# JinfengX/PointCloudPDF

Measured on AMD Instinct MI355X. Metric: points/sec fwd+bwd (PT-v1 Seg50 + PDF U-decoder, 100k-pt scenes), higher is better.
Workload: dtype f32

## Files before the change

### pointcloudpdf_amd/csrc/rowlin2_impl.h

```cpp
#pragma once
#include "pdfops_common.h"
#include <algorithm>
#include <cstdlib>

namespace rl2 {

typedef float f32x4 __attribute__((ext_vector_type(4)));

typedef _Float16 h16x4 __attribute__((ext_vector_type(4)));
typedef __bf16 b16x4 __attribute__((ext_vector_type(4)));
typedef short s16x4 __attribute__((ext_vector_type(4)));
template <int MP> struct Mma;
template <> struct Mma<0> {
    typedef f32x4 frag;
    static __device__ __forceinline__ frag cvt(f32x4 v) { return v; }
};
template <> struct Mma<1> {
    typedef h16x4 frag;
    static __device__ __forceinline__ frag cvt(f32x4 v) { return __builtin_convertvector(v, h16x4); }
    static __device__ __forceinline__ f32x4 mma(frag a, frag b, f32x4 acc) { return __builtin_amdgcn_mfma_f32_16x16x16f16(a, b, acc, 0, 0, 0); }
};
template <> struct Mma<2> {
    typedef s16x4 frag;
    static __device__ __forceinline__ frag cvt(f32x4 v) { return __builtin_bit_cast(s16x4, __builtin_convertvector(v, b16x4)); }
    static __device__ __forceinline__ f32x4 mma(frag a, frag b, f32x4 acc) { return __builtin_amdgcn_mfma_f32_16x16x16bf16_1k(a, b, acc, 0, 0, 0); }
};

long stats_rows_floats(long n, int o);

struct FwdArgs {
    long N;
    int O;
    const float *X[3]; long ldx;
    const float *W[3]; long wso, wsk;
    const float *bias[3];
    const float *scale, *shift; int relu;
    float *Y[3]; long ldy;
    int accumulate;
    float *partial;
    const float *bx; long ldb; const float *bcoef; int brelu;
    const float *roww; long rws;
    unsigned long long *ho_gran; unsigned *ho_sync;
};

constexpr int FWD_CAP = 1024;
static inline int fwd_row_blocks(long n) {
    const long tiles = (n + 15) / 16, b = (tiles + 3) / 4;
    return (int)(b < 1 ? 1 : (b > FWD_CAP ? FWD_CAP : b));
}

template <int K, int NOB, int NIN, bool PRE, int ST, int MP>
__global__ __launch_bounds__(256) void k_fwd(FwdArgs a) {
    typedef typename Mma<MP>::frag wfrag;
    constexpr bool STATS = ST != 0;
    constexpr int NJ = K / 16;
    constexpr bool COEF_REGS = K <= 64;
    const int lane = threadIdx.x & 63, wave = threadIdx.x >> 6;
    const int li = lane & 15, kq = lane >> 4;
    if (ST == 1 && a.ho_gran && blockIdx.x == 0 && blockIdx.y == 0) pdf_handoff_zero(a.ho_gran, a.O, a.ho_sync);
    const int gcol0 = blockIdx.y * NOB * 16;
    int outi[NOB], colb[NOB];
#pragma unroll
    for (int ob = 0; ob < NOB; ++ob) { outi[ob] = (gcol0 + ob * 16) / a.O; colb[ob] = gcol0 + ob * 16 - outi[ob] * a.O; }
    wfrag Wr[NIN][NOB][NJ];
#pragma unroll
    for (int in = 0; in < NIN; ++in) {
#pragma unroll
        for (int ob = 0; ob < NOB; ++ob) {
            const float *W = a.W[NIN > 1 ? in : outi[ob]];
            const long o = colb[ob] + li;
#pragma unroll
            for (int j = 0; j < NJ; ++j) {
                f32x4 w4;
                if (a.wsk == 1) {
                    w4 = *reinterpret_cast<const f32x4 *>(W + o * a.wso + 16 * j + 4 * kq);
                } else {
#pragma unroll
                    for (int c = 0; c < 4; ++c) w4[c] = W[o * a.wso + (long)(16 * j + 4 * kq + c) * a.wsk];
                }
                Wr[in][ob][j] = Mma<MP>::cvt(w4);
            }
        }
    }
    f32x4 bias4[NOB];
#pragma unroll
    for (int ob = 0; ob < NOB; ++ob) {
        const float *b = a.bias[NIN > 1 ? 0 : outi[ob]];
#pragma unroll
        for (int r = 0; r < 4; ++r) bias4[ob][r] = b ? b[colb[ob] + 4 * kq + r] : 0.f;
    }
    f32x4 sc4[COEF_REGS && PRE ? NJ : 1], sh4[COEF_REGS && PRE ? NJ : 1];
    if (PRE && COEF_REGS) {
#pragma unroll
        for (int j = 0; j < NJ; ++j) {
            sc4[j] = *reinterpret_cast<const f32x4 *>(a.scale + 16 * j + 4 * kq);
            sh4[j] = *reinterpret_cast<const f32x4 *>(a.shift + 16 * j + 4 * kq);
        }
    }
    f32x4 s4[STATS ? NOB : 1], ss4[STATS ? NOB : 1];
    if (STATS) {
#pragma unroll
        for (int ob = 0; ob < NOB; ++ob) { s4[ob] = f32x4{0.f, 0.f, 0.f, 0.f}; ss4[ob] = f32x4{0.f, 0.f, 0.f, 0.f}; }
    }
    __shared__ float bco[ST == 2 ? 3 : 1][NOB * 16];
    if (ST == 2) {
        if (threadIdx.x < 3 * NOB * 16) {
            const int v = threadIdx.x / (NOB * 16), t = threadIdx.x % (NOB * 16);
            bco[ST == 2 ? v : 0][t] = a.bcoef[(long)v * a.O + gcol0 + t];
        }
        __syncthreads();
    }
    __shared__ float pco[PRE && !COEF_REGS ? 2 : 1][PRE && !COEF_REGS ? K : 1];
    if (PRE && !COEF_REGS) {
        for (int t = threadIdx.x; t < K; t += 256) { pco[0][t] = a.scale[t]; pco[PRE && !COEF_REGS ? 1 : 0][t] = a.shift[t]; }
        __syncthreads();
    }
    const float relu_lo = a.relu ? 0.f : -INFINITY;
    constexpr int XB0 = NJ < 16 ? NJ : 16;
    constexpr int XB = (K == 256 && NIN == 3) ? 4 : ((ST != 0 && NOB > 1 && NIN * NOB * NJ * 4 >= 128) ? ((PRE && K == 128) ? 2 : XB0 / 2) : XB0);
    const long ntiles = (a.N + 15) / 16;
    for (long tile = (long)blockIdx.x * 4 + wave; tile < ntiles; tile += (long)gridDim.x * 4) {
        const long n = tile * 16 + li;
        const bool valid = n < a.N;
        f32x4 acc[NOB];
#pragma unroll
        for (int ob = 0; ob < NOB; ++ob) acc[ob] = f32x4{0.f, 0.f, 0.f, 0.f};
#pragma unroll
        for (int in = 0; in < NIN; ++in) {
            const float *xr = a.X[in] + (valid ? n : 0) * a.ldx + 4 * kq;
#pragma unroll
            for (int j0 = 0; j0 < NJ; j0 += XB) {
                f32x4 xb[XB];
#pragma unroll
                for (int t = 0; t < XB; ++t) xb[t] = *reinterpret_cast<const f32x4 *>(xr + 16 * (j0 + t));
                __builtin_amdgcn_sched_barrier(0);
#pragma unroll
                for (int t = 0; t < XB; ++t) {
                    const int j = j0 + t;
                    f32x4 x4 = xb[t];
                    if (PRE) {
                        const f32x4 sc = COEF_REGS ? sc4[COEF_REGS ? j : 0] : *reinterpret_cast<const f32x4 *>(&pco[0][16 * j + 4 * kq]);
                        const f32x4 sh = COEF_REGS ? sh4[COEF_REGS ? j : 0] : *reinterpret_cast<const f32x4 *>(&pco[PRE && !COEF_REGS ? 1 : 0][16 * j + 4 * kq]);
                        x4 = x4 * sc + sh;
#pragma unroll
                        for (int c = 0; c < 4; ++c) x4[c] = fmaxf(x4[c], relu_lo);
                    }
                    if constexpr (MP == 0) {
#pragma unroll
                        for (int c = 0; c < 4; ++c)
#pragma unroll
                            for (int ob = 0; ob < NOB; ++ob)
                                acc[ob] = __builtin_amdgcn_mfma_f32_16x16x4f32(Wr[in][ob][j][c], x4[c], acc[ob], 0, 0, 0);
                    } else {
                        const wfrag xh = Mma<MP>::cvt(x4);
#pragma unroll
                        for (int ob = 0; ob < NOB; ++ob) acc[ob] = Mma<MP>::mma(Wr[in][ob][j], xh, acc[ob]);
                    }
                }
            }
        }
#pragma unroll
        for (int ob = 0; ob < NOB; ++ob) {
            f32x4 v = acc[ob];
            if (a.roww) v *= a.roww[(valid ? n : 0) * a.rws];
            v += bias4[ob];
            float *dst = a.Y[outi[ob]] + (valid ? n : 0) * a.ldy + colb[ob] + 4 * kq;
            if (a.accumulate && valid) v += *reinterpret_cast<const f32x4 *>(dst);
            if (valid) *reinterpret_cast<f32x4 *>(dst) = v;
            if (ST == 1 && valid) { s4[ob] += v; ss4[ob] += v * v; }
            if (ST == 2) {
                const f32x4 x4 = *reinterpret_cast<const f32x4 *>(a.bx + (valid ? n : 0) * a.ldb + colb[ob] + 4 * kq);
                const f32x4 sc = *reinterpret_cast<const f32x4 *>(&bco[0][ob * 16 + 4 * kq]);
                const f32x4 sh = *reinterpret_cast<const f32x4 *>(&bco[ST == 2 ? 1 : 0][ob * 16 + 4 * kq]);
                const f32x4 mu = *reinterpret_cast<const f32x4 *>(&bco[ST == 2 ? 2 : 0][ob * 16 + 4 * kq]);
                const f32x4 pre = x4 * sc + sh;
                f32x4 gm;
#pragma unroll
                for (int c = 0; c < 4; ++c) gm[c] = (valid && (!a.brelu || pre[c] > 0.f)) ? v[c] : 0.f;
                s4[ob] += gm;
                ss4[ob] += gm * (x4 - mu);
            }
        }
    }
    if (STATS) {
        __shared__ float red[4][2][NOB * 16];
#pragma unroll
        for (int ob = 0; ob < NOB; ++ob)
#pragma unroll
            for (int r = 0; r < 4; ++r) {
                float s = s4[ob][r], ss = ss4[ob][r];
#pragma unroll
                for (int m = 1; m < 16; m <<= 1) { s += __shfl_xor(s, m, 64); ss += __shfl_xor(ss, m, 64); }
                if (li == 0) { red[wave][0][ob * 16 + 4 * kq + r] = s; red[wave][1][ob * 16 + 4 * kq + r] = ss; }
            }
        __syncthreads();
        const int t = threadIdx.x;
        if (t < NOB * 16) {
            float *row = a.partial + (size_t)blockIdx.x * 2 * a.O;
            row[gcol0 + t] = red[0][0][t] + red[1][0][t] + red[2][0][t] + red[3][0][t];
            const float ss = red[0][1][t] + red[1][1][t] + red[2][1][t] + red[3][1][t];
            row[a.O + gcol0 + t] = ST == 2 ? ss * a.bcoef[3 * (long)a.O + gcol0 + t] : ss;
        }
    }
}

constexpr int WG_MAXG = 5;
struct WArgs {
    long N;
    int K, O;
    const float *G[WG_MAXG]; long ldg;
    const float *X; long ldx;
    const float *scale, *shift; int relu;
    int per_z; const float *Xz[WG_MAXG]; const float *scalez[WG_MAXG], *shiftz[WG_MAXG]; int reluz[WG_MAXG];
    float *dW[WG_MAXG], *db[WG_MAXG];
    long rows_per_block;
    const float *roww; long rws;
    float *slab;
    float *bslab;
};

template <int VW> struct Vec;
template <> struct Vec<2> { typedef float type __attribute__((ext_vector_type(2))); };
template <> struct Vec<4> { typedef float type __attribute__((ext_vector_type(4))); };

template <int VW, bool PRE, bool RW, int MP>
__global__ __launch_bounds__(256) void k_wg(WArgs a) {
    typedef typename Vec<VW>::type vec;
    constexpr int B = 16 * VW;
    __shared__ float red[4][B * B];
    __shared__ float redb[4][B];
    const int lane = threadIdx.x & 63, wave = threadIdx.x >> 6;
    const int li = lane & 15, nq = lane >> 4;
    const int nkb = a.K / B;
    const int ob = (blockIdx.y / nkb) * B, kb = (blockIdx.y % nkb) * B;
    const float *G = a.G[blockIdx.z];
    const float *X = (PRE && a.per_z) ? a.Xz[blockIdx.z] : a.X;
    vec sc, sh;
    bool relu = a.relu != 0;
    if (PRE) {
        const float *scp = a.per_z ? a.scalez[blockIdx.z] : a.scale, *shp = a.per_z ? a.shiftz[blockIdx.z] : a.shift;
        if (a.per_z) relu = scp != nullptr && a.reluz[blockIdx.z] != 0;
        if (scp) {
            sc = *reinterpret_cast<const vec *>(scp + kb + VW * li);
            sh = *reinterpret_cast<const vec *>(shp + kb + VW * li);
        } else {
#pragma unroll
            for (int c = 0; c < VW; ++c) { sc[c] = 1.f; sh[c] = 0.f; }
        }
    }
    const float relu_lo = relu ? 0.f : -INFINITY;
    f32x4 acc[VW][VW];
    float gsum[VW];
#pragma unroll
    for (int c = 0; c < VW; ++c) {
        gsum[c] = 0.f;
#pragma unroll
        for (int c2 = 0; c2 < VW; ++c2) acc[c][c2] = f32x4{0.f, 0.f, 0.f, 0.f};
    }
    const long rb = (long)blockIdx.x * a.rows_per_block;
    const long re = rb + a.rows_per_block < a.N ? rb + a.rows_per_block : a.N;
    for (long r0 = rb + 16 * wave; r0 < re; r0 += 64) {
        vec gv[4], xv[4];
        float rw[RW ? 4 : 1];
        bool ok[4];
#pragma unroll
        for (int t = 0; t < 4; ++t) {
            const long n = r0 + 4 * t + nq;
            ok[t] = n < re;
            const long nn = ok[t] ? n : rb;
            gv[t] = *reinterpret_cast<const vec *>(G + nn * a.ldg + ob + VW * li);
            xv[t] = *reinterpret_cast<const vec *>(X + nn * a.ldx + kb + VW * li);
            if (RW) rw[RW ? t : 0] = a.roww[nn * a.rws];
        }
        __builtin_amdgcn_sched_barrier(0);
#pragma unroll
        for (int t = 0; t < 4; ++t) {
            if (RW) gv[t] *= rw[RW ? t : 0];
            if (PRE) {
                xv[t] = xv[t] * sc + sh;
#pragma unroll
                for (int c = 0; c < VW; ++c) xv[t][c] = fmaxf(xv[t][c], relu_lo);
            }
#pragma unroll
            for (int c = 0; c < VW; ++c) { gv[t][c] = ok[t] ? gv[t][c] : 0.f; xv[t][c] = ok[t] ? xv[t][c] : 0.f; }
        }
        if constexpr (MP == 0) {
#pragma unroll
            for (int t = 0; t < 4; ++t)
#pragma unroll
                for (int c = 0; c < VW; ++c) {
                    gsum[c] += gv[t][c];
#pragma unroll
                    for (int c2 = 0; c2 < VW; ++c2)
                        acc[c][c2] = __builtin_amdgcn_mfma_f32_16x16x4f32(gv[t][c], xv[t][c2], acc[c][c2], 0, 0, 0);
                }
        } else {
            typename Mma<MP>::frag ga[VW], xa[VW];
#pragma unroll
            for (int c = 0; c < VW; ++c) {
                gsum[c] += (gv[0][c] + gv[1][c]) + (gv[2][c] + gv[3][c]);
                ga[c] = Mma<MP>::cvt(f32x4{gv[0][c], gv[1][c], gv[2][c], gv[3][c]});
                xa[c] = Mma<MP>::cvt(f32x4{xv[0][c], xv[1][c], xv[2][c], xv[3][c]});
            }
#pragma unroll
            for (int c = 0; c < VW; ++c)
#pragma unroll
                for (int c2 = 0; c2 < VW; ++c2) acc[c][c2] = Mma<MP>::mma(ga[c], xa[c2], acc[c][c2]);
        }
    }
#pragma unroll
    for (int c = 0; c < VW; ++c)
#pragma unroll
        for (int c2 = 0; c2 < VW; ++c2)
#pragma unroll
            for (int r = 0; r < 4; ++r) red[wave][(VW * (4 * nq + r) + c) * B + VW * li + c2] = acc[c][c2][r];
    float *db = a.db[blockIdx.z];
    const bool want_db = db && kb == 0;
    if (want_db) {
#pragma unroll
        for (int c = 0; c < VW; ++c) {
            float g = gsum[c];
            g += __shfl_xor(g, 16, 64);
            g += __shfl_xor(g, 32, 64);
            if (nq == 0) redb[wave][VW * li + c] = g;
        }
    }
    __syncthreads();
    float *slab = a.slab + (((size_t)blockIdx.z * gridDim.y + blockIdx.y) * gridDim.x + blockIdx.x) * (B * B);
    for (int e = threadIdx.x; e < B * B; e += 256) slab[e] = (red[0][e] + red[1][e]) + (red[2][e] + red[3][e]);
    if (want_db && threadIdx.x < B)
        a.bslab[(((size_t)blockIdx.z * (a.O / B) + ob / B) * gridDim.x + blockIdx.x) * B + threadIdx.x] =
            (redb[0][threadIdx.x] + redb[1][threadIdx.x]) + (redb[2][threadIdx.x] + redb[3][threadIdx.x]);
}

struct RArgs {
    const float *slab, *bslab;
    float *dW[WG_MAXG], *db[WG_MAXG];
    int B, tiles_k, tiles, otiles, split, K, O;
};
void launch_slab_reduce(const RArgs &a, int ng, bool any_bias, hipStream_t s);
template <int L>
__global__ __launch_bounds__(64 * L) void k_slab_reduce(RArgs a) {
    __shared__ float red[L][64];
    const int e = threadIdx.x & 63, l = threadIdx.x >> 6, z = blockIdx.z;
    const int ei = blockIdx.x * 64 + e;
    const bool bias = (int)blockIdx.y >= a.tiles;
    const int t = bias ? (int)blockIdx.y - a.tiles : (int)blockIdx.y;
    const int len = bias ? a.B : a.B * a.B;
    if (bias && (int)blockIdx.x * 64 >= len) return;
    const float *src = bias ? a.bslab + ((size_t)z * a.otiles + t) * a.split * a.B : a.slab + ((size_t)z * a.tiles + t) * a.split * (size_t)(a.B * a.B);
    float s = 0.f;
    if (ei < len) {
        int k = l;
        for (; k + 3 * L < a.split; k += 4 * L) {
            const float v0 = src[(size_t)k * len + ei], v1 = src[(size_t)(k + L) * len + ei];
            const float v2 = src[(size_t)(k + 2 * L) * len + ei], v3 = src[(size_t)(k + 3 * L) * len + ei];
            s = (((s + v0) + v1) + v2) + v3;
        }
        for (; k < a.split; k += L) s += src[(size_t)k * len + ei];
    }
    red[l][e] = s;
    __syncthreads();
    if (l != 0 || ei >= len) return;
#pragma unroll
    for (int k = 1; k < L; ++k) s += red[k][e];
    if (bias) {
        const int o = t * a.B + ei;
        if (a.db[z] && o < a.O) a.db[z][o] = s;
    } else {
        const int o = (t / a.tiles_k) * a.B + ei / a.B, kk = (t % a.tiles_k) * a.B + ei % a.B;
        if (o < a.O && kk < a.K) a.dW[z][(size_t)o * a.K + kk] = s;
    }
}

#ifdef RL2_MAIN_TU
void launch_slab_reduce(const RArgs &a, int ng, bool any_bias, hipStream_t s) {
    const dim3 grid((unsigned)((a.B * a.B + 63) / 64), (unsigned)(a.tiles + (any_bias ? a.otiles : 0)), (unsigned)ng);
    if (a.split > 32) k_slab_reduce<16><<<grid, 64 * 16, 0, s>>>(a);
    else if (a.split > 4) k_slab_reduce<4><<<grid, 64 * 4, 0, s>>>(a);
    else k_slab_reduce<1><<<grid, 64, 0, s>>>(a);
}
#endif

struct WgPlan { int vw, b, nblk; long split, rows_per_block; };
static WgPlan wg_plan(long n, int k, int o, int ng) {
    WgPlan p;
    p.vw = (k % 64 == 0 && o % 64 == 0) ? 4 : ((k % 32 == 0 && o % 32 == 0) ? 2 : 0);
    p.b = 16 * p.vw;
    if (!p.vw) { p.nblk = 0; p.split = 0; p.rows_per_block = 0; return p; }
    p.nblk = (o / p.b) * (k / p.b) * ng;
    static const int target = [] { const char *v = getenv("PDFOPS_WG_BLOCKS"); const int x = v ? atoi(v) : 0; return x > 0 ? x : 512; }();
    long split = (target + p.nblk - 1) / p.nblk;
    const long max_split = (n + 255) / 256;
    if (split > max_split) split = max_split;
    if (split < 1) split = 1;
    p.rows_per_block = ((n + split - 1) / split + 63) / 64 * 64;
    p.split = (n + p.rows_per_block - 1) / p.rows_per_block;
    return p;
}
#ifdef RL2_MAIN_TU
long wgrad_ws_floats(long n, int k, int o, int ng) {
    const WgPlan p = wg_plan(n, k, o, ng);
    if (!p.vw) return 0;
    return (long)p.nblk * p.split * p.b * p.b + (long)ng * (o / p.b) * p.split * p.b;
}
#endif

static inline bool aligned16(const void *p) { return (reinterpret_cast<uintptr_t>(p) & 15) == 0; }

template <int K, int NOB, int NIN, int MP>
static int launch_fwd(const FwdArgs &a, int nslabs, hipStream_t s) {
    const bool pre = a.scale != nullptr, stats = a.partial != nullptr, bst = stats && a.bx != nullptr;
    static const int total = [] { const char *v = getenv("PDFOPS_RL_BLOCKS"); const int x = v ? atoi(v) : 0; return x > 0 ? x : 512; }();
    int gx = fwd_row_blocks(a.N);
    if (!stats || bst) gx = std::max(1, std::min(gx, std::max(8, total / std::max(nslabs, 1))));
    const dim3 grid((unsigned)gx, (unsigned)nslabs);
    if (bst) {
        k_fwd<K, NOB, NIN, false, 2, MP><<<grid, 256, 0, s>>>(a);
    } else if (NIN == 1 && stats) {
        if (pre) k_fwd<K, NOB, 1, true, 1, MP><<<grid, 256, 0, s>>>(a);
        else k_fwd<K, NOB, 1, false, 1, MP><<<grid, 256, 0, s>>>(a);
    } else {
        if (pre) k_fwd<K, NOB, NIN, true, 0, MP><<<grid, 256, 0, s>>>(a);
        else k_fwd<K, NOB, NIN, false, 0, MP><<<grid, 256, 0, s>>>(a);
    }
    return gx;
}

#ifdef RL2_MAIN_TU
long stats_rows_floats(long n, int o) { return (long)fwd_row_blocks(n) * 2 * o; }
#endif

template <int MP>
int try_forward_mp(long n, int k, int o, int nin, int nout, const float *const *x, long ldx, const float *const *w, int transpose_w,
                   const float *const *bias, const float *scale, const float *shift, int relu, float *const *y, long ldy,
                   int accumulate, float *partial, hipStream_t s, const float *roww, long rws, const float *bx, long ldb, const float *bcoef,
                   int brelu, int *partial_rows, long ldw, void *handoff) {
    if (nin < 1 || nout < 1 || (nin > 1 && nout > 1) || nin > 3 || nout > 3) return 0;
    if (nin == 2 && (scale || bx)) return 0;
    if (partial && !bx && (nin != 1 || nout != 1)) return 0;
    if (bx && (!partial || nout != 1 || scale || !bcoef || (ldb & 3) || !aligned16(bx) || !aligned16(bcoef))) return 0;
    if ((ldx & 3) || (ldy & 3) || (o & 15)) return 0;
    for (int i = 0; i < (nin > 1 ? nin : nout); ++i) if (!aligned16(w[i])) return 0;
    if (scale && (!aligned16(scale) || !aligned16(shift))) return 0;
    for (int i = 0; i < nin; ++i) if (!aligned16(x[i])) return 0;
    for (int i = 0; i < nout; ++i) if (!aligned16(y[i])) return 0;
    FwdArgs a;
    a.N = n; a.O = o; a.ldx = ldx; a.ldy = ldy; a.scale = scale; a.shift = shift; a.relu = relu; a.accumulate = accumulate;
    a.partial = partial; a.roww = roww; a.rws = rws;
    a.bx = bx; a.ldb = ldb; a.bcoef = bcoef; a.brelu = brelu;
    a.ho_gran = static_cast<unsigned long long *>(handoff);
    a.ho_sync = handoff ? reinterpret_cast<unsigned *>(a.ho_gran + 2 * (size_t)o) : nullptr;
    a.wso = transpose_w ? 1 : (ldw ? ldw : k); a.wsk = transpose_w ? o : 1;
    for (int i = 0; i < 3; ++i) {
        a.X[i] = i < nin ? x[i] : nullptr;
        a.W[i] = i < (nin > 1 ? nin : nout) ? w[i] : nullptr;
        a.bias[i] = (bias && i < nout) ? bias[i] : nullptr;
        a.Y[i] = i < nout ? y[i] : nullptr;
    }
    const int cols = o * nout;
#define PDF_RL2(K_, NOB_, NIN_) do { if (cols % (NOB_ * 16) == 0) { \
        const int r_ = launch_fwd<K_, NOB_, NIN_, MP>(a, cols / (NOB_ * 16), s); \
        if (partial_rows) *partial_rows = r_; \
        return 1; } } while (0)
    if (nin == 1) {
        switch (k) {
        case 32: if (!partial) PDF_RL2(32, 6, 1); PDF_RL2(32, 2, 1); PDF_RL2(32, 1, 1); break;
        case 64: PDF_RL2(64, 4, 1); PDF_RL2(64, 1, 1); break;
        case 128: if (!bx) PDF_RL2(128, 4, 1); else PDF_RL2(128, 2, 1); PDF_RL2(128, 1, 1); break;
        case 256: PDF_RL2(256, 2, 1); PDF_RL2(256, 1, 1); break;
        case 512: PDF_RL2(512, 1, 1); break;
        default: break;
        }
    } else if (nin == 2) {
        if (k == 512) PDF_RL2(512, 1, 2);
    } else if (nin == 3) {
        switch (k) {
        case 32: PDF_RL2(32, 2, 3); break;
        case 64: PDF_RL2(64, 2, 3); break;
        case 128: PDF_RL2(128, 1, 3); break;
        case 256: PDF_RL2(256, 1, 3); break;
        default: break;
        }
    }
#undef PDF_RL2
    return 0;
}

template <int MP>
int try_wgrad_mp(long n, int k, int o, int ng, const float *const *g, long ldg, const float *x, long ldx, const float *scale,
                 const float *shift, int relu, float *const *dw, float *const *db, float *ws, hipStream_t s, const float *roww, long rws) {
    if (ng < 1 || ng > 3 || !ws) return 0;
    const WgPlan p = wg_plan(n, k, o, ng);
    const int vw = p.vw;
    if (!vw) return 0;
    if ((ldg % vw) || (ldx % vw) || !aligned16(x)) return 0;
    if (scale && (!aligned16(scale) || !aligned16(shift))) return 0;
    for (int i = 0; i < ng; ++i) if (!aligned16(g[i])) return 0;
    WArgs a;
    a.N = n; a.K = k; a.O = o; a.ldg = ldg; a.X = x; a.ldx = ldx; a.scale = scale; a.shift = shift; a.relu = relu; a.roww = roww; a.rws = rws;
    a.per_z = 0;
    bool any_bias = false;
    for (int i = 0; i < WG_MAXG; ++i) {
        a.G[i] = i < ng ? g[i] : nullptr; a.dW[i] = i < ng ? dw[i] : nullptr; a.db[i] = (db && i < ng) ? db[i] : nullptr;
        a.Xz[i] = nullptr; a.scalez[i] = a.shiftz[i] = nullptr; a.reluz[i] = 0;
        any_bias = any_bias || a.db[i] != nullptr;
    }
    const int b = p.b;
    a.rows_per_block = p.rows_per_block;
    a.slab = ws;
    a.bslab = ws + (size_t)p.nblk * p.split * b * b;
    const dim3 grid((unsigned)p.split, (unsigned)((o / b) * (k / b)), (unsigned)ng);
#define PDF_WG(VW_) do { \
        if (roww) { if (scale) k_wg<VW_, true, true, MP><<<grid, 256, 0, s>>>(a); else k_wg<VW_, false, true, MP><<<grid, 256, 0, s>>>(a); } \
        else      { if (scale) k_wg<VW_, true, false, MP><<<grid, 256, 0, s>>>(a); else k_wg<VW_, false, false, MP><<<grid, 256, 0, s>>>(a); } } while (0)
    if (vw == 4) PDF_WG(4); else PDF_WG(2);
#undef PDF_WG
    RArgs r;
    r.slab = a.slab; r.bslab = a.bslab; r.B = b; r.tiles_k = k / b; r.tiles = (o / b) * (k / b); r.otiles = o / b; r.split = (int)p.split; r.K = k; r.O = o;
    for (int i = 0; i < WG_MAXG; ++i) { r.dW[i] = a.dW[i]; r.db[i] = a.db[i]; }
    launch_slab_reduce(r, ng, any_bias, s);
    return 1;
}

template <int MP>
int try_wgrad_group_mp(long n, int k, int o, int ng, const float *const *g, long ldg, const float *const *x, long ldx,
                       const float *const *scale, const float *const *shift, const int *relu, float *const *dw, float *const *db,
                       float *ws, hipStream_t s) {
    if (ng < 1 || ng > WG_MAXG || !ws) return 0;
    const WgPlan p = wg_plan(n, k, o, ng);
    const int vw = p.vw;
    if (!vw) return 0;
    if ((ldg % vw) || (ldx % vw)) return 0;
    for (int i = 0; i < ng; ++i) {
        if (!aligned16(g[i]) || !aligned16(x[i])) return 0;
        if (scale[i] && (!aligned16(scale[i]) || !aligned16(shift[i]))) return 0;
    }
    WArgs a;
    a.N = n; a.K = k; a.O = o; a.ldg = ldg; a.X = nullptr; a.ldx = ldx; a.scale = a.shift = nullptr; a.relu = 0; a.roww = nullptr; a.rws = 0;
    a.per_z = 1;
    bool any_bias = false;
    for (int i = 0; i < WG_MAXG; ++i) {
        const bool on = i < ng;
        a.G[i] = on ? g[i] : nullptr; a.Xz[i] = on ? x[i] : nullptr;
        a.scalez[i] = on ? scale[i] : nullptr; a.shiftz[i] = on ? shift[i] : nullptr; a.reluz[i] = on ? relu[i] : 0;
        a.dW[i] = on ? dw[i] : nullptr; a.db[i] = (on && db) ? db[i] : nullptr;
        any_bias = any_bias || a.db[i] != nullptr;
    }
    const int b = p.b;
    a.rows_per_block = p.rows_per_block;
    a.slab = ws;
    a.bslab = ws + (size_t)p.nblk * p.split * b * b;
    const dim3 grid((unsigned)p.split, (unsigned)((o / b) * (k / b)), (unsigned)ng);
    if (vw == 4) k_wg<4, true, false, MP><<<grid, 256, 0, s>>>(a); else k_wg<2, true, false, MP><<<grid, 256, 0, s>>>(a);
    RArgs r;
    r.slab = a.slab; r.bslab = a.bslab; r.B = b; r.tiles_k = k / b; r.tiles = (o / b) * (k / b); r.otiles = o / b; r.split = (int)p.split; r.K = k; r.O = o;
    for (int i = 0; i < WG_MAXG; ++i) { r.dW[i] = a.dW[i]; r.db[i] = a.db[i]; }
    launch_slab_reduce(r, ng, any_bias, s);
    return 1;
}

#ifdef RL2_MAIN_TU
int stats_rows(long n) { return fwd_row_blocks(n); }
#endif

}
```

Baseline: 13.36 million.

## Add grouped-column forward kernel staging weights in LDS for small-N wide-K layers

Adds a k_fwd_group kernel that splits output columns into groups of two 16-column blocks per workgroup. Each group's weights are staged once in dynamic LDS, and row tiles are streamed with double-buffered input loads. It is used when N is at most 16384 rows and K is at least 128, so small-row layers get more column-parallel blocks and less weight reloading. The cost is a large dynamic LDS footprint that needs a raised limit, with fallback to the slab kernel if that fails, plus extra template instantiations and an env override.

```diff
diff --git a/pointcloudpdf_amd/csrc/rowlin2_impl.h b/pointcloudpdf_amd/csrc/rowlin2_impl.h
--- a/pointcloudpdf_amd/csrc/rowlin2_impl.h
+++ b/pointcloudpdf_amd/csrc/rowlin2_impl.h
@@ -2,6 +2,7 @@
 #include "pdfops_common.h"
 #include <algorithm>
 #include <cstdlib>
+#include <cstring>
 
 namespace rl2 {
 
@@ -200,6 +201,156 @@
             row[gcol0 + t] = red[0][0][t] + red[1][0][t] + red[2][0][t] + red[3][0][t];
             const float ss = red[0][1][t] + red[1][1][t] + red[2][1][t] + red[3][1][t];
             row[a.O + gcol0 + t] = ST == 2 ? ss * a.bcoef[3 * (long)a.O + gcol0 + t] : ss;
+        }
+    }
+}
+
+constexpr int GROUP_GN = 2;
+template <int K, int GN, int NIN, int MP> constexpr int group_lds_bytes() { return NIN * GN * (K / 16) * 64 * (int)sizeof(typename Mma<MP>::frag); }
+
+template <int K, int GN, int NIN, bool PRE, int ST, int MP>
+__global__ __launch_bounds__(256, 2) void k_fwd_group(FwdArgs a) {
+    typedef typename Mma<MP>::frag wfrag;
+    constexpr bool STATS = ST != 0;
+    constexpr int NJ = K / 16;
+    static_assert(K >= 128 && NJ % 8 == 0 && (NIN == 1 || NIN == 3), "group form: K = 128 / 256 / 512, one or three inputs");
+    extern __shared__ __attribute__((aligned(16))) unsigned char group_lds[];
+    wfrag *Wl = reinterpret_cast<wfrag *>(group_lds);
+    const int lane = threadIdx.x & 63, wave = threadIdx.x >> 6;
+    const int li = lane & 15, kq = lane >> 4;
+    if (ST == 1 && a.ho_gran && blockIdx.x == 0 && blockIdx.y == 0) pdf_handoff_zero(a.ho_gran, a.O, a.ho_sync);
+    const int gcol0 = blockIdx.y * GN * 16;
+    int outi[GN], colb[GN];
+#pragma unroll
+    for (int ob = 0; ob < GN; ++ob) { outi[ob] = (gcol0 + ob * 16) / a.O; colb[ob] = gcol0 + ob * 16 - outi[ob] * a.O; }
+    {
+        constexpr int PER_WAVE = NIN * GN * NJ / 4;
+        f32x4 w4[PER_WAVE];
+#pragma unroll
+        for (int t = 0; t < PER_WAVE; ++t) {
+            const int f = t * 4 + wave;
+            const int j = f % NJ, ob = (f / NJ) % GN, in = f / (NJ * GN);
+            const int col = gcol0 + ob * 16, oi = col / a.O;
+            const float *W = a.W[NIN > 1 ? in : oi];
+            const long o = col - oi * a.O + li;
+            if (a.wsk == 1) {
+                w4[t] = *reinterpret_cast<const f32x4 *>(W + o * a.wso + 16 * j + 4 * kq);
+            } else {
+#pragma unroll
+                for (int c = 0; c < 4; ++c) w4[t][c] = W[o * a.wso + (long)(16 * j + 4 * kq + c) * a.wsk];
+            }
+        }
+#pragma unroll
+        for (int t = 0; t < PER_WAVE; ++t) Wl[(t * 4 + wave) * 64 + lane] = Mma<MP>::cvt(w4[t]);
+    }
+    __shared__ float bco[ST == 2 ? 3 : 1][GN * 16];
+    if (ST == 2 && threadIdx.x < 3 * GN * 16) {
+        const int v = threadIdx.x / (GN * 16), t = threadIdx.x % (GN * 16);
+        bco[ST == 2 ? v : 0][t] = a.bcoef[(long)v * a.O + gcol0 + t];
+    }
+    __shared__ float pco[PRE ? 2 : 1][PRE ? K : 1];
+    if (PRE)
+        for (int t = threadIdx.x; t < K; t += 256) { pco[0][t] = a.scale[t]; pco[PRE ? 1 : 0][t] = a.shift[t]; }
+    __syncthreads();
+    f32x4 s4[STATS ? GN : 1], ss4[STATS ? GN : 1];
+    if (STATS) {
+#pragma unroll
+        for (int ob = 0; ob < GN; ++ob) { s4[ob] = f32x4{0.f, 0.f, 0.f, 0.f}; ss4[ob] = f32x4{0.f, 0.f, 0.f, 0.f}; }
+    }
+    const float relu_lo = a.relu ? 0.f : -INFINITY;
+    constexpr int XB = 8, NBJ = NJ / XB, NB = NIN * NBJ;
+    const long ntiles = (a.N + 15) / 16;
+    for (long tile = (long)blockIdx.x * 4 + wave; tile < ntiles; tile += (long)gridDim.x * 4) {
+        const long n = tile * 16 + li;
+        const bool valid = n < a.N;
+        const long row = valid ? n : 0;
+        f32x4 acc[GN];
+#pragma unroll
+        for (int ob = 0; ob < GN; ++ob) acc[ob] = f32x4{0.f, 0.f, 0.f, 0.f};
+        f32x4 xb[2][XB];
+#pragma unroll
+        for (int t = 0; t < XB; ++t) xb[0][t] = *reinterpret_cast<const f32x4 *>(a.X[0] + row * a.ldx + 4 * kq + 16 * t);
+#pragma unroll
+        for (int b = 0; b < NB; ++b) {
+            if (b + 1 < NB) {
+                const float *xr = a.X[(b + 1) / NBJ] + row * a.ldx + 4 * kq + 16 * ((b + 1) % NBJ) * XB;
+#pragma unroll
+                for (int t = 0; t < XB; ++t) xb[(b + 1) & 1][t] = *reinterpret_cast<const f32x4 *>(xr + 16 * t);
+            }
+            __builtin_amdgcn_sched_barrier(0);
+            const int in = b / NBJ;
+#pragma unroll
+            for (int t = 0; t < XB; ++t) {
+                const int j = (b % NBJ) * XB + t;
+                f32x4 x4 = xb[b & 1][t];
+                if (PRE) {
+                    const f32x4 sc = *reinterpret_cast<const f32x4 *>(&pco[0][16 * j + 4 * kq]);
+                    const f32x4 sh = *reinterpret_cast<const f32x4 *>(&pco[PRE ? 1 : 0][16 * j + 4 * kq]);
+                    x4 = x4 * sc + sh;
+#pragma unroll
+                    for (int c = 0; c < 4; ++c) x4[c] = fmaxf(x4[c], relu_lo);
+                }
+                wfrag wa[GN];
+#pragma unroll
+                for (int ob = 0; ob < GN; ++ob) wa[ob] = Wl[((in * GN + ob) * NJ + j) * 64 + lane];
+                if constexpr (MP == 0) {
+#pragma unroll
+                    for (int c = 0; c < 4; ++c)
+#pragma unroll
+                        for (int ob = 0; ob < GN; ++ob)
+                            acc[ob] = __builtin_amdgcn_mfma_f32_16x16x4f32(wa[ob][c], x4[c], acc[ob], 0, 0, 0);
+                } else {
+                    const wfrag xh = Mma<MP>::cvt(x4);
+#pragma unroll
+                    for (int ob = 0; ob < GN; ++ob) acc[ob] = Mma<MP>::mma(wa[ob], xh, acc[ob]);
+                }
+            }
+        }
+#pragma unroll
+        for (int ob = 0; ob < GN; ++ob) {
+            f32x4 v = acc[ob];
+            if (a.roww) v *= a.roww[row * a.rws];
+            const float *bp = a.bias[NIN > 1 ? 0 : outi[ob]];
+            f32x4 bias4;
+#pragma unroll
+            for (int r = 0; r < 4; ++r) bias4[r] = bp ? bp[colb[ob] + 4 * kq + r] : 0.f;
+            v += bias4;
+            float *dst = a.Y[outi[ob]] + row * a.ldy + colb[ob] + 4 * kq;
+            if (a.accumulate && valid) v += *reinterpret_cast<const f32x4 *>(dst);
+            if (valid) *reinterpret_cast<f32x4 *>(dst) = v;
+            if (ST == 1 && valid) { s4[ob] += v; ss4[ob] += v * v; }
+            if (ST == 2) {
+                const f32x4 x4 = *reinterpret_cast<const f32x4 *>(a.bx + row * a.ldb + colb[ob] + 4 * kq);
+                const f32x4 sc = *reinterpret_cast<const f32x4 *>(&bco[0][ob * 16 + 4 * kq]);
+                const f32x4 sh = *reinterpret_cast<const f32x4 *>(&bco[ST == 2 ? 1 : 0][ob * 16 + 4 * kq]);
+                const f32x4 mu = *reinterpret_cast<const f32x4 *>(&bco[ST == 2 ? 2 : 0][ob * 16 + 4 * kq]);
+                const f32x4 pre = x4 * sc + sh;
+                f32x4 gm;
+#pragma unroll
+                for (int c = 0; c < 4; ++c) gm[c] = (valid && (!a.brelu || pre[c] > 0.f)) ? v[c] : 0.f;
+                s4[ob] += gm;
+                ss4[ob] += gm * (x4 - mu);
+            }
+        }
+    }
+    if (STATS) {
+        __shared__ float red[4][2][GN * 16];
+#pragma unroll
+        for (int ob = 0; ob < GN; ++ob)
+#pragma unroll
+            for (int r = 0; r < 4; ++r) {
+                float s = s4[ob][r], ss = ss4[ob][r];
+#pragma unroll
+                for (int m = 1; m < 16; m <<= 1) { s += __shfl_xor(s, m, 64); ss += __shfl_xor(ss, m, 64); }
+                if (li == 0) { red[wave][0][ob * 16 + 4 * kq + r] = s; red[wave][1][ob * 16 + 4 * kq + r] = ss; }
+            }
+        __syncthreads();
+        const int t = threadIdx.x;
+        if (t < GN * 16) {
+            float *prow = a.partial + (size_t)blockIdx.x * 2 * a.O;
+            prow[gcol0 + t] = red[0][0][t] + red[1][0][t] + red[2][0][t] + red[3][0][t];
+            const float ss = red[0][1][t] + red[1][1][t] + red[2][1][t] + red[3][1][t];
+            prow[a.O + gcol0 + t] = ST == 2 ? ss * a.bcoef[3 * (long)a.O + gcol0 + t] : ss;
         }
     }
 }
@@ -408,12 +559,45 @@
 
 static inline bool aligned16(const void *p) { return (reinterpret_cast<uintptr_t>(p) & 15) == 0; }
 
+constexpr long GROUP_MAX_ROWS = 16384;
+static bool group_form_wanted(const FwdArgs &a, int k, int blocks) {
+    if (blocks % GROUP_GN) return false;
+    if (const char *f = getenv("PDFOPS_RL_FORM")) {
+        if (!strcmp(f, "slab")) return false;
+        if (!strcmp(f, "group")) return true;
+    }
+    return a.N <= GROUP_MAX_ROWS && !(k == 128 && blocks * 16 > a.O);
+}
+
+template <int K, int GN, int NIN, bool PRE, int ST, int MP>
+static bool launch_group_kernel(const FwdArgs &a, dim3 grid, hipStream_t s) {
+    constexpr int lds = group_lds_bytes<K, GN, NIN, MP>();
+    static PdfLdsLimit site;
+    if (!pdf_lds_limit_raised(site, reinterpret_cast<const void *>(&k_fwd_group<K, GN, NIN, PRE, ST, MP>), lds)) return false;
+    k_fwd_group<K, GN, NIN, PRE, ST, MP><<<grid, 256, lds, s>>>(a);
+    return true;
+}
+
+template <int K, int GN, int NIN, int MP>
+static bool launch_fwd_group(const FwdArgs &a, int blocks, int gx, hipStream_t s) {
+    const bool pre = a.scale != nullptr, stats = a.partial != nullptr, bst = stats && a.bx != nullptr;
+    const dim3 grid((unsigned)gx, (unsigned)(blocks / GN));
+    if (bst) return launch_group_kernel<K, GN, NIN, false, 2, MP>(a, grid, s);
+    if constexpr (NIN == 1) {
+        if (stats) return pre ? launch_group_kernel<K, GN, 1, true, 1, MP>(a, grid, s) : launch_group_kernel<K, GN, 1, false, 1, MP>(a, grid, s);
+    }
+    return pre ? launch_group_kernel<K, GN, NIN, true, 0, MP>(a, grid, s) : launch_group_kernel<K, GN, NIN, false, 0, MP>(a, grid, s);
+}
+
 template <int K, int NOB, int NIN, int MP>
 static int launch_fwd(const FwdArgs &a, int nslabs, hipStream_t s) {
     const bool pre = a.scale != nullptr, stats = a.partial != nullptr, bst = stats && a.bx != nullptr;
     static const int total = [] { const char *v = getenv("PDFOPS_RL_BLOCKS"); const int x = v ? atoi(v) : 0; return x > 0 ? x : 512; }();
     int gx = fwd_row_blocks(a.N);
     if (!stats || bst) gx = std::max(1, std::min(gx, std::max(8, total / std::max(nslabs, 1))));
+    if constexpr (K >= 128 && NIN != 2) {
+        if (group_form_wanted(a, K, nslabs * NOB) && launch_fwd_group<K, GROUP_GN, NIN, MP>(a, nslabs * NOB, gx, s)) return gx;
+    }
     const dim3 grid((unsigned)gx, (unsigned)nslabs);
     if (bst) {
         k_fwd<K, NOB, NIN, false, 2, MP><<<grid, 256, 0, s>>>(a);
```

After: 13.70 million, median of 6. 2.6% higher.
